# Danya-Is/re2-modification

Measured on AMD Instinct MI355X. Metric: input GB/s (chars matched/sec) on 10-example attack corpus, higher is better.
Workload: dtype u8

## Files before the change

### re2-modification_amd/csrc/walk.h

```cpp
#ifndef MFA_WALK_H
#define MFA_WALK_H

#include <cstddef>
#include <cstdint>

#ifndef WALK_MIN_WAVES
#define WALK_MIN_WAVES 2
#endif

namespace mfa {

constexpr uint32_t WALK_MAX_SEG = 16;
constexpr uint32_t WALK_LDS_BYTES = 160u * 1024u;
constexpr uint32_t CMP_CACHE = 4;
#define MFA_RT_CACHED 2u

constexpr uint32_t walk_W(uint32_t K) { return 2u + 2u * K; }
constexpr uint32_t walk_DW(uint32_t K) { return (1u + 2u * K + 1u) / 2u; }

struct WalkLayout {
    uint32_t K, C, CX;
    bool images_global;
    bool lean;
    uint32_t nm_words;
// ... 19 lines not shown
};
constexpr size_t walk_lds_bytes(uint32_t shared_words, const WalkLayout& l) { return ((size_t)shared_words + 4u * (size_t)l.lds_words()) * sizeof(uint32_t); }

struct WalkArgs {
    const uint8_t*  bytes;
    const uint64_t* offsets;
    uint64_t        n;
    uint8_t*        results;
    const uint64_t* regions;
    const uint32_t* tables;
    uint32_t*       spill;
    unsigned long long* counter;
    uint32_t table_words, shared_words;
    uint32_t n_seg, C, CX, accel, refill;
    uint32_t images_global;
    uint32_t nm_words;
    uint32_t* lean_queue;
    uint32_t* lean_seen;
    uint32_t seg_first[WALK_MAX_SEG + 1];
    uint32_t seg_table[WALK_MAX_SEG];
};

constexpr uint32_t WALK_MAX_K = 9;
enum class WalkKernel { plain, long_k1, stats };

struct WalkLaunch {
    WalkArgs args;
    uint32_t K;
    WalkKernel kernel;
    unsigned grid;
// ... 23 lines not shown
```

### re2-modification_amd/csrc/walk.hip

```cpp
#include <hip/hip_runtime.h>

#include "mfa_internal.h"
#include "walk.h"
#include "walk_core.h"

#ifndef WALK_STATS
#define WALK_STATS 0
#endif
#ifndef WALK_K
#error "compile with -DWALK_K=<cells>"
#endif

namespace mfa {

using namespace mfa_walk;

struct TicketFeeder {
    unsigned long long* counter;
    uint64_t n, first_sid;
    bool first_round = true;
    __device__ __forceinline__ bool take(bool want, uint64_t& sid) {
        const uint32_t lane = threadIdx.x & 63u;
        const unsigned long long wb = __ballot(want);
        unsigned long long first = 0;
// ... 18 lines not shown
    if (!TG) {
        for (uint32_t k = threadIdx.x; k < a.table_words; k += blockDim.x) smem[k] = a.tables[k];
        __syncthreads();
    }
    const WalkLayout lay{(uint32_t)K, a.C, a.CX, a.images_global != 0u, false, WALK_NODE_MAP ? a.nm_words : 0u};
    const uint32_t wave_u = (uint32_t)__builtin_amdgcn_readfirstlane((int)wave);
    WALK_LDS uint32_t* const base = (WALK_LDS uint32_t*)smem + a.shared_words + wave_u * lay.lds_words();
    Store st;
    st.C = a.C; st.CX = a.CX; st.CI = lay.CI();
    st.lv = base + lay.lv(); st.ld = base + lay.ld(); st.sb = base + lay.sb(); st.sa = base + lay.sa();
    WALK_LDS uint64_t* const rtc = (WALK_LDS uint64_t*)(base + lay.rtc());
    st.nm = (WALK_LDS uint8_t*)(base + lay.nm()); st.nm_words = lay.nm_words;
    const uint64_t gwave = (uint64_t)blockIdx.x * 4u + wave_u;
    uint32_t* const g = a.spill + gwave * lay.spill_words();
    st.gv = g + lay.gv(); st.gd = g + lay.gd(); st.gsb = g + lay.gsb(); st.gsa = g + lay.gsa(); st.gq = g + lay.gq();
    Batch b{a.bytes, a.offsets, a.n, a.results, a.regions, a.accel, a.refill, a.n_seg, a.seg_first, a.seg_table, 0u,
            a.lean_queue, reinterpret_cast<uint32_t*>(a.counter + 1)};
    TicketFeeder feed{a.counter, a.n, gwave * 64u};
#if WALK_STATS
    WaveStats ws;
    if (TG) walk_wave<K, REV, TicketFeeder, TablePtrG>(b, a.tables, st, rtc, feed, &ws);
    else walk_wave<K, REV, TicketFeeder, TablePtr>(b, (TablePtr)smem, st, rtc, feed, &ws);
    unsigned long long* out = a.counter + 8;
    const unsigned long long lanev[7] = {ws.dual * 0ull + ws.skipped, ws.probes, ws.hits, ws.steps, ws.spills, ws.strings, 0ull};
    for (int k = 0; k < 6; k++) atomicAdd(&out[k], lanev[k]);
    if ((threadIdx.x & 63u) == 0) {
        const unsigned long long wavev[9] = {ws.iters, ws.dual, ws.t_start, ws.t_byte, ws.t_look, ws.t_plain, ws.t_dual, ws.t_post, ws.t_total};
        for (int k = 0; k < 9; k++) atomicAdd(&out[8 + k], wavev[k]);
        atomicAdd(&out[17], 1ull);
    }
#else
    if (TG) walk_wave<K, REV, TicketFeeder, TablePtrG>(b, a.tables, st, rtc, feed, nullptr);
    else walk_wave<K, REV, TicketFeeder, TablePtr>(b, (TablePtr)smem, st, rtc, feed, nullptr);
#endif
}

struct QueueFeeder {
    const uint32_t* queue;
    uint32_t count;
    unsigned long long* counter;
    __device__ __forceinline__ bool take(bool want, uint64_t& sid) {
        const uint32_t lane = threadIdx.x & 63u;
        const unsigned long long wb = __ballot(want);
        const int leader = __builtin_ctzll(wb);
        unsigned long long first = 0;
        if (lane == (uint32_t)leader) first = atomicAdd(counter, (unsigned long long)__builtin_popcountll(wb));
        const uint32_t at = (uint32_t)__shfl((uint32_t)first, leader) + (uint32_t)__builtin_popcountll(wb & ((1ull << lane) - 1ull));
        const bool got = want && at < count;
// ... 14 lines not shown
        __syncthreads();
    }
    const WalkLayout lay{(uint32_t)K, a.C, a.CX, false, true, WALK_NODE_MAP ? a.nm_words : 0u};
    const uint32_t wave_u = (uint32_t)__builtin_amdgcn_readfirstlane((int)(threadIdx.x >> 6));
    WALK_LDS uint32_t* const base = (WALK_LDS uint32_t*)smem + a.shared_words + wave_u * lay.lds_words();
    Store st;
    st.C = a.C; st.CX = a.CX; st.CI = 0u;
    st.lv = base + lay.lv();
    st.nm = (WALK_LDS uint8_t*)(base + lay.nm()); st.nm_words = lay.nm_words;
    st.ld = nullptr; st.sb = nullptr; st.sa = nullptr;
    const uint64_t gwave = (uint64_t)blockIdx.x * 4u + wave_u;
    uint32_t* const g = a.spill + gwave * lay.spill_words();
    st.gv = g + lay.gv();
    st.gd = nullptr; st.gsb = nullptr; st.gsa = nullptr;
    st.gq = g + lay.gq();
    Batch b{a.bytes, a.offsets, a.n, a.results, nullptr, 0u, a.refill, a.n_seg, a.seg_first, a.seg_table, 0u, nullptr, nullptr};
    QueueFeeder feed{a.lean_queue, count, a.counter + 2};
    if (TG) walk_wave_lean<K, REV, QueueFeeder, TablePtrG>(b, a.tables, st, feed);
    else walk_wave_lean<K, REV, QueueFeeder, TablePtr>(b, (TablePtr)smem, st, feed);
}

#define WALK_CAT2(a, b) a##b
#define WALK_CAT(a, b) WALK_CAT2(a, b)

#if WALK_STATS
int launch_walk_stats(const WalkLaunch& L, void* stream) {
#elif defined(WALK_LONG_LISTS)
int WALK_CAT(launch_walk_long_k, WALK_K)(const WalkLaunch& L, void* stream) {
#else
int WALK_CAT(launch_walk_k, WALK_K)(const WalkLaunch& L, void* stream) {
#endif
// ... 35 lines not shown
```

### re2-modification_amd/csrc/walk_core.h

```cpp
#ifndef MFA_WALK_CORE_H
#define MFA_WALK_CORE_H

#include "../../include/mfa_image_format.h"
#define MFA_SCAN_DEPTH 1
#define MFA_RUN_DEPTH 1
#include "device_common.h"
#include "walk.h"

#ifndef WALK_WV
#define WALK_WV 64u
#endif
#ifndef WALK_DEV
#define WALK_DEV __device__ __forceinline__
#endif
#ifndef WALK_WITH_DUAL
#define WALK_WITH_DUAL 1
#endif
#ifndef WALK_PROBE_PERIODS
#define WALK_PROBE_PERIODS 5u
#endif
#ifndef WALK_NODE_MAP
#define WALK_NODE_MAP 0
#endif
#ifndef WALK_LEAN_MIN_LEN
// ... 10 lines not shown
#define VI_CACC  4u
#define VI_QUAL  8u
#define VI_HASC  (1u << 17)

#define TIE_CARRY 0u
#define TIE_HERE  1u
#define TIE_WAIT  1025u

#ifdef MFA_HOST_EMUL
static unsigned long long g_ev[8];
#define WALK_EV(k) (g_ev[k]++)
WALK_DEV uint32_t wv_lane() { return 0u; }
WALK_DEV uint64_t wv_shfl64(uint64_t v, int) { return v; }
WALK_DEV uint32_t wv_atomic_add(uint32_t* p, uint32_t v) { const uint32_t o = *p; *p = o + v; return o; }
WALK_DEV uint32_t wv_bcast32(uint32_t v, int) { return v; }
template <bool REV>
inline uint32_t coop_run_end_x(const uint8_t* bytes, uint64_t base, uint32_t len, uint32_t i0, uint32_t) {
    if (i0 + 1u >= len) return len;
    auto at = [&](uint32_t j) { return bytes[base + (REV ? (uint64_t)(len - 1u - j) : (uint64_t)j)]; };
    const uint8_t c = at(i0);
    uint32_t j = i0 + 1u;
    while (j < len && at(j) == c) j++;
    return j;
}
inline bool coop_mem_equal_x(const uint8_t* bytes, uint64_t pa, uint64_t pb, uint32_t l, uint32_t) {
    for (uint32_t k = 0; k < l; k++)
        if (bytes[pa + k] != bytes[pb + k]) return false;
    return true;
}
#else
#define WALK_EV(k) ((void)0)
WALK_DEV uint32_t wv_lane() { return threadIdx.x & 63u; }
WALK_DEV uint32_t wv_atomic_add(uint32_t* p, uint32_t v) { return atomicAdd(p, v); }
WALK_DEV uint32_t wv_bcast32(uint32_t v, int L) { return (uint32_t)__shfl((int)v, L); }
WALK_DEV uint64_t wv_shfl64(uint64_t v, int L) { return ((uint64_t)__shfl((uint32_t)(v >> 32), L) << 32) | __shfl((uint32_t)v, L); }
template <bool REV>
__device__ __attribute__((noinline)) uint32_t coop_run_end_x(const uint8_t* bytes, uint64_t base, uint32_t len, uint32_t i0, uint32_t lane) { return coop_run_end<REV>(bytes, base, len, i0, lane); }
__device__ __attribute__((noinline)) bool coop_mem_equal_x(const uint8_t* bytes, uint64_t pa, uint64_t pb, uint32_t l, uint32_t lane) { return coop_mem_equal(bytes, pa, pb, l, lane); }
#endif

#ifdef MFA_HOST_EMUL
#define WALK_LDS
#else
#define WALK_LDS __attribute__((address_space(3)))
#endif
typedef const WALK_LDS uint32_t* TablePtr;
typedef const uint32_t* TablePtrG;

struct WIn {
    const uint8_t*  bytes;
    uint64_t        total16;
    const uint64_t* regions;
    WALK_LDS uint64_t* rtc;
    uint64_t base;
    uint32_t len, sid;
    uint64_t blk;
    uint32_t w0, w1, w2, w3;
    uint32_t run_lo, run_hi, run_ch;
    uint32_t per_lo, per_hi, per_q;
    uint32_t prev_lo, prev_hi, prev_q;
    uint32_t dual_p;
    uint32_t rt_cnt;
    uint32_t rq;
    uint32_t rq_a, rq_b, rq_l;
    uint32_t cq_n;
};

WALK_DEV void w_drop_window(WIn& in) { in.blk = MFA_NO_WINDOW; }
WALK_DEV void w_reset(WIn& in, uint64_t base, uint32_t len, uint32_t sid) {
    in.base = base; in.len = len; in.sid = sid;
    w_drop_window(in);
    in.run_lo = in.run_hi = 0; in.run_ch = 0x100u;
    in.per_lo = in.per_hi = 0; in.per_q = 0; in.dual_p = 0;
    in.prev_lo = in.prev_hi = 0; in.prev_q = 0;
    in.rt_cnt = 0; in.rq = 0; in.rq_a = in.rq_b = in.rq_l = 0; in.cq_n = 0;
}

WALK_DEV void w_rt_attach(WIn& in, uint32_t& warm, const uint4 a, const uint4 b) {
    if (in.regions == nullptr) return;
    const uint32_t lane = wv_lane();
// ... 539 lines not shown
        }
}
#endif

template <int K, class TP>
WALK_DEV void ee_decode(TP T, uint32_t at, bool p, uint32_t& e0, uint32_t& actions, uint32_t& cm, uint32_t& com, uint32_t& rdm) {
    e0 = p ? T[at] : 0u;
    const uint32_t e1 = p ? T[at + 1] : 0u;
    if (Lay<K>::EEW == 2) {
        actions = e1 & 0xfffu; cm = (e1 >> 12) & 0x3fu; com = (e1 >> 18) & 0x3fu; rdm = (e1 >> 24) & 0x3fu;
    } else {
        const uint32_t e2 = p ? T[at + 2] : 0u;
        actions = e1 & 0x3ffffu; cm = (e1 >> 18) & 0x1ffu; com = e2 & 0x1ffu; rdm = (e2 >> 9) & 0x1ffu;
    }
}

template <class U, int K>
WALK_DEV void frame_state(const Ent<U, K>& E, U pos, uint32_t cm, uint32_t com, uint32_t rdm, Ent<U, K>& s) {
#pragma unroll
    for (int c = 0; c < K; c++) {
        const bool created = (cm >> c) & 1u;
        s.S[c] = sel(created, pos, E.S[c]);
        s.L[c] = sel(created, konst<U>(0u), E.L[c]);
        s.F[c] = created ? (F_PRESENT | F_UNI | (((com >> c) & 1u) ? F_OPEN : 0u)) : E.F[c];
        if ((rdm >> c) & 1u) s.F[c] |= F_READ;
    }
}

#ifndef WALK_STEP_ATTR
#define WALK_STEP_ATTR WALK_DEV
#endif
template <class U, int K, bool REV, class TP>
WALK_STEP_ATTR void walk_step(const Store& st, TP T, const Aut& au, WIn& in, uint32_t cur, uint32_t n_cur, uint32_t& n_next,
                        const U i, const U len, const uint32_t ch, const bool final_pass, const bool active, const bool dual_lane,
                        bool& accept, bool& fits, tb_t& TB, uint32_t& shape) {
    StepCtx<U, K> cx{st, cur ^ 1u, 0u, dual_lane, fits, TB, {}};
    cx.keys.seen = 0ull;
    uint32_t sh = 0u;
#pragma unroll
    for (uint32_t k = 0; k < KeyCache<U>::N; k++) cx.keys.id[k] = 0xffffffffu;
    const uint32_t cls = (active && !final_pass) ? (T[au.cmap() + ((ch & 0xffu) >> 2)] >> (8u * (ch & 3u))) & 0xffu : 0u;
    for (uint32_t e = 0; __any(active && e < n_cur); e++) {
        const bool have = active && e < n_cur;
        if (have) WALK_EV(0);
        Ent<U, K> E;
        load_entry<U, K>(st, cur, have ? e : 0u, dual_lane && have, E);
        const U pos = have ? posof(E.P, cx.TB) : konst<U>(0u);
        bool live = have && ge(pos, i, cx.TB);
        if (REV) {
            if (live) {
                U need = konst<U>(0u);
#pragma unroll
                for (int c = 0; c < K; c++)
                    if ((E.F[c] & F_PRESENT) && ((E.F[c] & F_OPEN) || !(E.F[c] & F_READ))) need = add(need, E.L[c]);
                live = le(need, sub(len, i), cx.TB);
            }
        }
        const bool here = live && !final_pass && eq(pos, i, cx.TB);
        const bool wait = live && !final_pass && !here;
        const uint32_t vi = have ? T[au.vinfo() + E.vid] : 0u;
        const uint32_t node = E.vid >> au.vbits();
#if WALK_NODE_MAP
        if (have) {
            WALK_LDS uint8_t* const mp = st.nm + nm_at(node);
            if (*mp == (uint8_t)((cur << 7) | e)) *mp = 0xffu;
        }
#endif
        if (have) {
            const uint32_t ahead = val(pos) - val(i);
            sh = ((sh << 7) | (sh >> 25)) ^ (E.vid * 4u + (ahead < 3u ? ahead : 3u) + 0x9e37u);
        }
        if ((vi & VI_EPS) && live && !accept && eq(pos, len, cx.TB)) accept = true;
        {
            const bool carry = wait && (vi & VI_QUAL) != 0u;
            if (__any(carry)) { Ent<U, K> t = E; insert<U, K>(cx, carry, E.vid, au.vbits(), E.P, TIE_CARRY, t); }
        }
        if (__any(here)) {
            const uint32_t bl = here ? T[au.vb() + E.vid * au.nc() + cls] : 0u;
            const uint32_t bbeg = bl >> 12, bcnt = bl & 0xfffu;
            for (uint32_t j = 0; __any(j < bcnt); j++) {
                const bool p = here && j < bcnt;
                if (p) WALK_EV(1);
                uint32_t e0, actions, cm, com, rdm;
                ee_decode<K, TP>(T, au.ee() + (bbeg + j) * Lay<K>::EEW, p, e0, actions, cm, com, rdm);
                const uint32_t tvid = e0 >> 9, tfn = (e0 >> 5) & 15u, cell = (e0 >> 1) & 15u;
                Ent<U, K> t = E;
                if (__any(p && (cm | rdm) != 0u)) frame_state<U, K>(E, pos, cm, com, rdm, t);
                const bool lit = p && (e0 & 1u) == 0u, rd = p && (e0 & 1u) != 0u;
                if (__any(lit)) {
                    apply_actions<U, K>(t, actions, lit, i, konst<U>(1u), true, ch, cx.TB);
                    insert<U, K>(cx, lit, tvid, au.vbits(), mkp(add(i, konst<U>(1u)), tfn), TIE_HERE + node, t);
                }
                if (__any(rd)) {
                    U vs = konst<U>(0u), vl = konst<U>(0u);
                    uint32_t vf = 0u;
#pragma unroll
                    for (int c = 0; c < K; c++)
                        if ((uint32_t)c == cell) { vs = t.S[c]; vl = t.L[c]; vf = t.F[c]; }
                    const bool ok = cell_read<REV, U>(st, in, rd, i, ch, vs, vl, vf, cx.TB);
                    if (__any(ok)) {
                        apply_actions<U, K>(t, actions, ok, i, vl, (vf & F_UNI) != 0u, (vf >> 8) & 0xffu, cx.TB);
                        insert<U, K>(cx, ok, tvid, au.vbits(), mkp(add(i, vl), tfn), TIE_HERE + node, t);
                    }
                }
            }
        }
        const bool late = live && !here;
        if ((vi & VI_CACC) && late && !accept && eq(pos, len, cx.TB)) accept = true;
        if (__any(wait && (vi & VI_HASC) != 0u)) {
            const uint32_t cl = (wait && (vi & VI_HASC) != 0u) ? T[au.vc() + E.vid] : 0u;
            const uint32_t cbeg = cl >> 12, ccnt = cl & 0xfffu;
            for (uint32_t j = 0; __any(j < ccnt); j++) {
                const bool p = wait && j < ccnt;
                if (p) WALK_EV(6);
                uint32_t e0, actions, cm, com, rdm;
                ee_decode<K, TP>(T, au.ee() + (cbeg + j) * Lay<K>::EEW, p, e0, actions, cm, com, rdm);
                Ent<U, K> t;
                frame_state<U, K>(E, pos, cm, com, 0u, t);
                insert<U, K>(cx, p, e0 >> 9, au.vbits(), mkp(pos, (e0 >> 5) & 15u), TIE_WAIT + node, t);
            }
        }
    }
    n_next = cx.n_next; fits = cx.fits; TB = cx.TB; shape = sh;
}

template <int K> WALK_DEV void sb_rd_words(const Store& st, uint32_t e, uint32_t (&w)[Lay<K>::W]) {
    if (e < st.CI) {
        const WALK_LDS uint32_t* p = st.sb + (e * Lay<K>::W) * WALK_WV + wv_lane();
#pragma unroll
        for (uint32_t k = 0; k < Lay<K>::W; k++) w[k] = p[k * WALK_WV];
    } else {
        const uint32_t* p = st.gsb + (size_t)((e - st.CI) * Lay<K>::W) * WALK_WV + wv_lane();
#pragma unroll
        for (uint32_t k = 0; k < Lay<K>::W; k++) w[k] = p[k * WALK_WV];
    }
}
template <int K> WALK_DEV void sb_wr_words(const Store& st, uint32_t e, const uint32_t (&w)[Lay<K>::W]) {
    if (e < st.CI) {
// ... 133 lines not shown
    const uint64_t* regions;
    uint32_t accel;
    uint32_t refill;
    uint32_t n_seg;
    const uint32_t* seg_first;
    const uint32_t* seg_table;
    uint32_t reserved;
    uint32_t* lean_queue;
    uint32_t* lean_count;
};

struct WaveStats {
    unsigned long long iters = 0, dual = 0, skipped = 0, probes = 0, hits = 0, steps = 0, spills = 0;
    unsigned long long t_start = 0, t_byte = 0, t_look = 0, t_plain = 0, t_dual = 0, t_post = 0, t_total = 0;
    unsigned long long strings = 0;
#ifdef MFA_HOST_EMUL
    unsigned long long hist[80] = {0};
#endif
};
#ifdef MFA_HOST_EMUL
WALK_DEV unsigned long long wv_clock() { return 0ull; }
#else
WALK_DEV unsigned long long wv_clock() { return __builtin_readcyclecounter(); }
#endif

struct ProbeCtl {
    uint32_t w;
    WALK_DEV uint32_t get(uint32_t sh, uint32_t bits) const { return (w >> sh) & ((1u << bits) - 1u); }
    WALK_DEV void put(uint32_t sh, uint32_t bits, uint32_t v) { w = (w & ~(((1u << bits) - 1u) << sh)) | ((v & ((1u << bits) - 1u)) << sh); }
    WALK_DEV void reset() { w = 0u; set_pp(1u); backoff_reset(); }
// ... 32 lines not shown
    }
    WALK_DEV uint32_t period(uint32_t q, uint32_t pmin) const {
        const uint32_t c = (uint32_t)(h >> 60);
        uint32_t m = 0u;
#pragma unroll
        for (uint32_t p = 1; p <= HIST_MAX_P; p++)
            if (((h ^ (h >> (5u * p))) & 1023ull) == 0ull) m |= 1u << p;
        const uint64_t lo = 0xffffull | (0x5555ull << 16) | (0x9249ull << 32) | (0x1111ull << 48), hi = 0x8421ull | (0x1041ull << 16) | (0x4081ull << 32) | (0x0101ull << 48);
        m &= (uint32_t)((q <= 4u ? lo : hi) >> (((q - 1u) & 3u) << 4)) & 0xffffu;
        m &= c >= 3u ? (1u << (c - 1u)) - 2u : 0u;
        m &= ~((1u << (pmin < 16u ? pmin : 16u)) - 1u);
        return m ? (uint32_t)__builtin_ctz(m) : 0u;
    }
};

template <int K, bool REV, class Feeder, class TP>
WALK_DEV void walk_wave(const Batch& b, TP T, const Store& st, WALK_LDS uint64_t* rt_cache, Feeder& feed, WaveStats* stats) {
    WIn in;
    in.bytes = b.bytes; in.total16 = (b.offsets[b.n] + 15u) & ~(uint64_t)15; in.regions = b.regions; in.rtc = rt_cache;
    w_reset(in, 0, 0, 0);
    in.w0 = in.w1 = in.w2 = in.w3 = 0;
    bool active = false, exhausted = false, accept = false;
    uint32_t i = 0, len = 0;
    uint32_t probe_at = 0;
    ProbeCtl P;
    P.reset();
    ShapeHist hist;
    hist.reset();
    tb_t TBacc = tb_init();
    bool fits = true, stable = false, patient = false;
    uint32_t cur = 0, n_cur = 0, sb_n = 0, warm = 0;
    Aut au;
    aut_load(au, T, 0u);
    const unsigned long long tm_begin = stats ? wv_clock() : 0ull;
    for (;;) {
        unsigned long long tm = stats ? wv_clock() : 0ull;
// ... 99 lines not shown
        }
        WALK_LAP(t_look);
        uint32_t n_next = 0, shape = 0;
        tb_t TB = tb_init();
        const bool p2 = P.phase() == 2u;
        const bool accept_before = accept, fits_before = fits;
        in.cq_n = 0u;
        for (;;) {
            n_next = 0; TB = tb_init(); accept = accept_before; fits = fits_before;
            if (WALK_WITH_DUAL && __any(p2)) {
                if (stats) stats->dual++;
                const Dual di{i, (int32_t)P.pp()}, dlen{len, 0};
                in.dual_p = p2 ? P.pp() : 0u;
                (void)lt(di, Dual{p2 ? in.per_hi : i + 1u, 0}, TB);
                (void)eq(di, dlen, TB);
                walk_step<Dual, K, REV, TP>(st, T, au, in, cur, n_cur, n_next, di, dlen, ch, final_pass, active, p2, accept, fits, TB, shape);
                in.dual_p = 0u;
                WALK_LAP(t_dual);
            } else {
                bool f2 = true;
                walk_step<uint32_t, K, REV, TP>(st, T, au, in, cur, n_cur, n_next, i, len, ch, final_pass, active, false, accept, f2, TB, shape);
                WALK_LAP(t_plain);
            }
            if (!__any(active && in.rq != 0u)) break;
            answer_requests<REV>(st, in, active);
#if WALK_NODE_MAP
            map_forget<K>(st, au.vbits(), cur ^ 1u, active, n_next);
#endif
        }
        cur ^= 1u;
        if (active) { n_cur = n_next; hist.push(shape); }
        const bool any_next = n_next != 0u;
        if (stats && active && n_cur > st.C) stats->spills++;
#ifdef MFA_HOST_EMUL
        if (stats && active) stats->hist[n_cur < 79u ? n_cur : 79u]++;
#endif
// ... 70 lines not shown
            }
        }
        if (active) {
            const bool done = accept || final_pass || !any_next;
            i++;
            if (stats) stats->steps++;
            if (done) {
                b.results[in.sid] = (warm == 0x9e3779b9u && len == 0xffffffffu) ? 3 : (accept ? 1 : 0);
                active = false; P.set_phase(0u); P.set_chain(0u); n_cur = 0u;
                if (stats) stats->strings++;
            }
        }
        WALK_LAP(t_post);
    }
#undef WALK_LAP
    if (stats) stats->t_total += wv_clock() - tm_begin;
}

template <int K, bool REV, class Feeder, class TP>
WALK_DEV void walk_wave_lean(const Batch& b, TP T, const Store& st, Feeder& feed) {
    WIn in;
    in.bytes = b.bytes; in.total16 = (b.offsets[b.n] + 15u) & ~(uint64_t)15; in.regions = nullptr; in.rtc = nullptr;
    w_reset(in, 0, 0, 0);
    in.w0 = in.w1 = in.w2 = in.w3 = 0;
    bool active = false, exhausted = false, accept = false;
    uint32_t i = 0, len = 0, cur = 0, n_cur = 0;
    Aut au;
    aut_load(au, T, 0u);
    for (;;) {
        {
            const bool want = !active && !exhausted;
            const unsigned long long wantb = __ballot(want);
            if (wantb && ((uint32_t)__builtin_popcountll(wantb) >= b.refill || !__any(active))) {
                uint64_t s = 0;
                const bool got = feed.take(want, s);
                if (want) {
                    if (!got) exhausted = true;
                    else {
                        const uint64_t o0 = b.offsets[s], o1 = b.offsets[s + 1];
                        len = (uint32_t)(o1 - o0);
                        w_reset(in, o0, len, (uint32_t)s);
                        uint32_t seg = 0;
                        for (uint32_t k = 1; k < b.n_seg; k++)
                            if (s >= b.seg_first[k]) seg = k;
                        aut_load(au, T, b.n_seg ? b.seg_table[seg] : 0u);
                        i = 0; accept = false; active = true;
#if WALK_NODE_MAP
                        for (uint32_t k = 0; k < st.nm_words; k++) reinterpret_cast<WALK_LDS uint32_t*>(st.nm)[k * WALK_WV + wv_lane()] = 0xffffffffu;
#endif
                        n_cur = 1;
                        Ent<uint32_t, K> e0;
                        e0.P = 0u; e0.vid = aut_start(T, au);
#pragma unroll
                        for (int c = 0; c < K; c++) { e0.S[c] = 0u; e0.L[c] = 0u; e0.F[c] = 0u; }
                        bool f2 = true;
                        store_entry<uint32_t, K>(st, cur, 0u, e0, 0u, f2);
                    }
                }
            }
        }
        if (!__any(active)) break;
        const bool final_pass = (i == len);
        uint32_t ch = 0x100u;
        if (active && !final_pass) ch = w_stream_byte<REV>(in, i);
        uint32_t n_next = 0, shape = 0;
        const bool accept_before = accept;
        in.cq_n = 0u;
        for (;;) {
            n_next = 0; accept = accept_before;
            tb_t TB = tb_init();
            bool f2 = true;
            walk_step<uint32_t, K, REV, TP>(st, T, au, in, cur, n_cur, n_next, i, len, ch, final_pass, active, false, accept, f2, TB, shape);
            if (!__any(active && in.rq != 0u)) break;
            answer_requests<REV>(st, in, active);
#if WALK_NODE_MAP
            map_forget<K>(st, au.vbits(), cur ^ 1u, active, n_next);
#endif
        }
        cur ^= 1u;
        if (active) {
            n_cur = n_next;
            const bool done = accept || final_pass || n_next == 0u;
            i++;
            if (done) { b.results[in.sid] = accept ? 1 : 0; active = false; n_cur = 0u; }
        }
    }
}
// ... 5 lines not shown
```

### re2-modification_amd/csrc/walk_launch.hip

```cpp
#include <hip/hip_runtime.h>

#include <algorithm>
#include <cstdio>
#include <cstdlib>
#include <cstring>
#include <map>
#include <new>
#include <string>
#include <vector>

#include "dfa_mixed.h"
#include "mfa_internal.h"
#include "walk.h"

namespace mfa {

int launch_walk(const WalkPlanInput& p, const uint32_t* d_tables, int n_cus, const uint8_t* d_bytes, const uint64_t* d_offsets, uint64_t n,
                uint8_t* d_results, const uint64_t* d_regions, uint32_t n_seg, const uint32_t* seg_first, const uint32_t* seg_table,
                uint32_t** d_spill, size_t* spill_bytes, unsigned long long* d_counter, void* stream, LeanHint* lean, void* wait_event) {
    if (n == 0) { if (wait_event) HIP_TRY(hipStreamWaitEvent((hipStream_t)stream, (hipEvent_t)wait_event, 0)); return MFA_OK; }
    const WalkKnobs kn = walk_knobs();
    Lean decision = d_regions != nullptr && kn.accel && kn.lean != 0 ? Lean::on : Lean::off;
    LeanHint next;
    const bool hinted = decision == Lean::on && lean != nullptr;
// ... 32 lines not shown

void lean_hint_free(LeanHint& h) {
    if (h.h_seen) (void)hipHostFree(h.h_seen);
    h.h_seen = nullptr;
}

void walk_print_stats(unsigned long long* d_counter, const char* tag) {
    unsigned long long h[32] = {0};
    if (hipMemcpy(h, d_counter, sizeof h, hipMemcpyDeviceToHost) != hipSuccess) return;
    const unsigned long long* o = h + 8;
    const double tot = (double)o[16] > 0 ? (double)o[16] : 1.0;
    fprintf(stderr, "%s stats: %llu waves, %llu strings, wave-iterations %llu (dual %llu), lane steps %llu, skipped %llu, probes %llu (hits %llu), spill steps %llu\n", tag,
            o[17], o[5], o[8], o[9], o[3], o[0], o[1], o[2], o[4]);
    fprintf(stderr, "%s stats: cycles per wave-iteration %.0f; share: string start %.1f%%, byte %.1f%%, region look-up %.1f%%, plain step %.1f%%, dual step %.1f%%, book-keeping %.1f%%\n", tag,
            tot / (double)(o[8] ? o[8] : 1), 100.0 * o[10] / tot, 100.0 * o[11] / tot, 100.0 * o[12] / tot, 100.0 * o[13] / tot, 100.0 * o[14] / tot, 100.0 * o[15] / tot);
}

}

using namespace mfa;

constexpr uint32_t MIX_TIMINGS = 32;

struct mfa_mixed {
    std::vector<mfa_image*> images;
    std::vector<uint32_t>   words;
    std::vector<uint32_t>   block_at;
    uint32_t K = 1, max_live = 1;
    bool reversed = false, table_ok = true;
    std::vector<uint8_t>    is_dfa, dfa_eligible, dfa_tables;
// ... 374 lines not shown
```

### re2-modification_amd/csrc/walk_plan.h

```cpp
#ifndef MFA_WALK_PLAN_H
#define MFA_WALK_PLAN_H

#include <algorithm>
#include <cmath>
#include <cstdint>
#include <cstdlib>
#include <string>
#include <vector>

#include "../../include/mfa_hip.h"
#include "walk.h"

namespace mfa {

inline int env_int(const char* name, int dflt) {
    const char* e = getenv(name);
    return e && *e ? atoi(e) : dflt;
}
inline bool env_is_off(const char* name) { const char* e = getenv(name); return e && e[0] == '0'; }
inline bool regions_enabled() { return !env_is_off("MFA_REGIONS") && !env_is_off("MFA_ACCEL"); }

inline int walk_mode() {
    const char* e = getenv("MFA_WALK");
    return !e ? 0 : e[0] == 't' ? 1 : e[0] == 'j' ? 2 : 0;
}

struct WalkPlanInput { uint32_t K, max_live; bool reversed; uint32_t table_words; };

struct LeanHint {
    uint32_t* h_seen = nullptr;
    uint32_t quiet = 0, launches = 0;
};
enum class Lean { off, on, probe };

struct WalkKnobs {
    bool tables_global, images_global, accel, long_lists, stats;
    int refill, want_c, wgs, waves_per_cu, grid_pct, spill_mb, lean;
};
inline WalkKnobs walk_knobs() {
    WalkKnobs k;
    k.tables_global = getenv("MFA_WALK_TABLES_GLOBAL") != nullptr;
    k.images_global = env_int("MFA_WALK_IMAGES_GLOBAL", 0) != 0;
    k.accel = !env_is_off("MFA_ACCEL");
    k.long_lists = env_int("MFA_WALK_LONG", 1) != 0;
    k.stats = getenv("MFA_WALK_STATS") != nullptr;
    k.refill = std::max(1, std::min(64, env_int("MFA_WALK_REFILL", 1)));
    k.want_c = env_int("MFA_WALK_C", 0);
    k.wgs = env_int("MFA_WALK_WGS", 0);
    k.waves_per_cu = env_int("MFA_WALK_WAVES_PER_CU", 0);
    k.grid_pct = env_int("MFA_WALK_GRID_PCT", 100);
    k.spill_mb = std::max(1, env_int("MFA_WALK_SPILL_MB", 2048));
    k.lean = env_int("MFA_WALK_LEAN", 1);
    return k;
}

inline Lean lean_decide(uint32_t seen, LeanHint& h, const WalkKnobs& kn) {
    h.quiet = seen == 1u ? h.quiet + 1u : 0u;
    Lean d = Lean::on;
    if (h.quiet >= 1u && kn.lean != 2) d = (h.launches & 31u) != 0u ? Lean::off : Lean::probe;
    h.launches++;
    return d;
}

inline int plan_walk(const WalkPlanInput& p, const WalkKnobs& kn, uint64_t n, int n_cus, uint32_t n_seg, Lean lean, WalkLaunch& L) {
    if (n_seg == 0 || n_seg > WALK_MAX_SEG || n > 0xffffffffull) return MFA_ERR_INVALID_ARG;
    L = WalkLaunch{};
    WalkArgs& a = L.args;
    a.n = n; a.n_seg = n_seg;
    a.table_words = p.table_words;
    a.shared_words = (p.table_words + 63u) & ~63u;
    const size_t lds_max = WALK_LDS_BYTES / 4u;
    L.tables_global = a.shared_words > lds_max / 3u || kn.tables_global;
    if (L.tables_global) a.shared_words = 0;
    a.accel = kn.accel ? 1u : 0u;
    a.refill = (uint32_t)kn.refill;
    a.images_global = kn.images_global ? 1u : 0u;
    L.K = p.K; L.reversed = p.reversed;
    const bool long_lists = p.K == 1 && p.max_live > 16u && p.max_live < 128u && kn.long_lists && !kn.stats;
    L.kernel = kn.stats && p.K == 1 ? WalkKernel::stats : long_lists ? WalkKernel::long_k1 : WalkKernel::plain;
    a.nm_words = long_lists ? (p.max_live + 1u + 3u) / 4u : 0u;
    const auto layout = [&](uint32_t C, bool lean_walk) { return WalkLayout{p.K, C, p.max_live > C ? p.max_live - C : 1u, kn.images_global, lean_walk, a.nm_words}; };
    const auto lds_words = [&](uint32_t C) { return (size_t)a.shared_words + 4u * (size_t)layout(C, false).lds_words(); };
    const uint64_t cus = (uint64_t)(n_cus > 0 ? n_cus : 256), want = (n + 255) / 256;
    const uint32_t wgs_goal = kn.wgs != 0 ? (uint32_t)kn.wgs : want <= cus ? 1u : 2u;
    uint32_t C = std::max(1u, std::min(p.max_live, kn.want_c > 0 ? (uint32_t)kn.want_c : 8u));
    while (C > 1 && kn.want_c <= 0 && lds_words(C) > lds_max / wgs_goal) C--;
    while (C > 1 && lds_words(C) > lds_max) C--;
    if (lds_words(C) > lds_max) return MFA_ERR_UNSUPPORTED;
    const WalkLayout full = layout(C, false), lean_lay = layout(C, true);
// ... 164 lines not shown
```

Baseline: 5270.

## Add wave-uniform scalar step path when all lanes share state and class

Before each step, the code checks with ballots whether every active lane has the same automaton, the same byte class and the same list of vertex ids. If they do, it runs a specialised path that broadcasts the ids and reads table entries with readfirstlane, so the loads become scalar and the loop bounds are uniform. The goal is to cut divergent vector table lookups and per-lane loop control. The main kernel keeps the general path unless WALK_UNIFORM_MAIN is set, so only the lean kernel takes the new path by default, and it pays for the uniformity check on every step even when lanes differ.

Result: no change. 5265 (-0.1%).

```diff
diff --git a/re2-modification_amd/csrc/walk.h b/re2-modification_amd/csrc/walk.h
--- a/re2-modification_amd/csrc/walk.h
+++ b/re2-modification_amd/csrc/walk.h
@@ -57,6 +57,7 @@
     uint32_t table_words, shared_words;
     uint32_t n_seg, C, CX, accel, refill;
     uint32_t images_global;
+    uint32_t flags;
     uint32_t nm_words;
     uint32_t* lean_queue;
     uint32_t* lean_seen;
diff --git a/re2-modification_amd/csrc/walk.hip b/re2-modification_amd/csrc/walk.hip
--- a/re2-modification_amd/csrc/walk.hip
+++ b/re2-modification_amd/csrc/walk.hip
@@ -6,6 +6,9 @@
 
 #ifndef WALK_STATS
 #define WALK_STATS 0
+#endif
+#ifndef WALK_UNIFORM_MAIN
+#define WALK_UNIFORM_MAIN WALK_STATS
 #endif
 #ifndef WALK_K
 #error "compile with -DWALK_K=<cells>"
@@ -56,13 +59,13 @@
     const uint64_t gwave = (uint64_t)blockIdx.x * 4u + wave_u;
     uint32_t* const g = a.spill + gwave * lay.spill_words();
     st.gv = g + lay.gv(); st.gd = g + lay.gd(); st.gsb = g + lay.gsb(); st.gsa = g + lay.gsa(); st.gq = g + lay.gq();
-    Batch b{a.bytes, a.offsets, a.n, a.results, a.regions, a.accel, a.refill, a.n_seg, a.seg_first, a.seg_table, 0u,
+    Batch b{a.bytes, a.offsets, a.n, a.results, a.regions, a.accel, a.refill, a.n_seg, a.seg_first, a.seg_table, a.flags & 1u,
             a.lean_queue, reinterpret_cast<uint32_t*>(a.counter + 1)};
     TicketFeeder feed{a.counter, a.n, gwave * 64u};
 #if WALK_STATS
     WaveStats ws;
-    if (TG) walk_wave<K, REV, TicketFeeder, TablePtrG>(b, a.tables, st, rtc, feed, &ws);
-    else walk_wave<K, REV, TicketFeeder, TablePtr>(b, (TablePtr)smem, st, rtc, feed, &ws);
+    if (TG) walk_wave<K, REV, TicketFeeder, TablePtrG, WALK_UNIFORM_MAIN != 0>(b, a.tables, st, rtc, feed, &ws);
+    else walk_wave<K, REV, TicketFeeder, TablePtr, WALK_UNIFORM_MAIN != 0>(b, (TablePtr)smem, st, rtc, feed, &ws);
     unsigned long long* out = a.counter + 8;
     const unsigned long long lanev[7] = {ws.dual * 0ull + ws.skipped, ws.probes, ws.hits, ws.steps, ws.spills, ws.strings, 0ull};
     for (int k = 0; k < 6; k++) atomicAdd(&out[k], lanev[k]);
@@ -70,10 +73,12 @@
         const unsigned long long wavev[9] = {ws.iters, ws.dual, ws.t_start, ws.t_byte, ws.t_look, ws.t_plain, ws.t_dual, ws.t_post, ws.t_total};
         for (int k = 0; k < 9; k++) atomicAdd(&out[8 + k], wavev[k]);
         atomicAdd(&out[17], 1ull);
+        atomicAdd(&out[18], ws.ent_uni);
+        atomicAdd(&out[19], ws.ent_gen);
     }
 #else
-    if (TG) walk_wave<K, REV, TicketFeeder, TablePtrG>(b, a.tables, st, rtc, feed, nullptr);
-    else walk_wave<K, REV, TicketFeeder, TablePtr>(b, (TablePtr)smem, st, rtc, feed, nullptr);
+    if (TG) walk_wave<K, REV, TicketFeeder, TablePtrG, WALK_UNIFORM_MAIN != 0>(b, a.tables, st, rtc, feed, nullptr);
+    else walk_wave<K, REV, TicketFeeder, TablePtr, WALK_UNIFORM_MAIN != 0>(b, (TablePtr)smem, st, rtc, feed, nullptr);
 #endif
 }
 
@@ -118,7 +123,7 @@
     st.gv = g + lay.gv();
     st.gd = nullptr; st.gsb = nullptr; st.gsa = nullptr;
     st.gq = g + lay.gq();
-    Batch b{a.bytes, a.offsets, a.n, a.results, nullptr, 0u, a.refill, a.n_seg, a.seg_first, a.seg_table, 0u, nullptr, nullptr};
+    Batch b{a.bytes, a.offsets, a.n, a.results, nullptr, 0u, a.refill, a.n_seg, a.seg_first, a.seg_table, a.flags & 1u, nullptr, nullptr};
     QueueFeeder feed{a.lean_queue, count, a.counter + 2};
     if (TG) walk_wave_lean<K, REV, QueueFeeder, TablePtrG>(b, a.tables, st, feed);
     else walk_wave_lean<K, REV, QueueFeeder, TablePtr>(b, (TablePtr)smem, st, feed);
diff --git a/re2-modification_amd/csrc/walk_core.h b/re2-modification_amd/csrc/walk_core.h
--- a/re2-modification_amd/csrc/walk_core.h
+++ b/re2-modification_amd/csrc/walk_core.h
@@ -48,6 +48,8 @@
 WALK_DEV uint64_t wv_shfl64(uint64_t v, int) { return v; }
 WALK_DEV uint32_t wv_atomic_add(uint32_t* p, uint32_t v) { const uint32_t o = *p; *p = o + v; return o; }
 WALK_DEV uint32_t wv_bcast32(uint32_t v, int) { return v; }
+WALK_DEV uint32_t wv_read_lane(uint32_t v, int) { return v; }
+template <bool UNI> WALK_DEV uint32_t wv_uni(uint32_t v) { return v; }
 template <bool REV>
 inline uint32_t coop_run_end_x(const uint8_t* bytes, uint64_t base, uint32_t len, uint32_t i0, uint32_t) {
     if (i0 + 1u >= len) return len;
@@ -68,10 +70,14 @@
 WALK_DEV uint32_t wv_atomic_add(uint32_t* p, uint32_t v) { return atomicAdd(p, v); }
 WALK_DEV uint32_t wv_bcast32(uint32_t v, int L) { return (uint32_t)__shfl((int)v, L); }
 WALK_DEV uint64_t wv_shfl64(uint64_t v, int L) { return ((uint64_t)__shfl((uint32_t)(v >> 32), L) << 32) | __shfl((uint32_t)v, L); }
+WALK_DEV uint32_t wv_read_lane(uint32_t v, int L) { return (uint32_t)__builtin_amdgcn_readlane((int)v, L); }
+template <bool UNI> WALK_DEV uint32_t wv_uni(uint32_t v) { return UNI ? (uint32_t)__builtin_amdgcn_readfirstlane((int)v) : v; }
 template <bool REV>
 __device__ __attribute__((noinline)) uint32_t coop_run_end_x(const uint8_t* bytes, uint64_t base, uint32_t len, uint32_t i0, uint32_t lane) { return coop_run_end<REV>(bytes, base, len, i0, lane); }
 __device__ __attribute__((noinline)) bool coop_mem_equal_x(const uint8_t* bytes, uint64_t pa, uint64_t pb, uint32_t l, uint32_t lane) { return coop_mem_equal(bytes, pa, pb, l, lane); }
 #endif
+
+template <bool UNI> WALK_DEV bool wv_any(bool c) { return UNI ? c : __any(c) != 0; }
 
 #ifdef MFA_HOST_EMUL
 #define WALK_LDS
@@ -98,6 +104,7 @@
     uint32_t rq;
     uint32_t rq_a, rq_b, rq_l;
     uint32_t cq_n;
+    uint32_t ev_uni, ev_gen;
 };
 
 WALK_DEV void w_drop_window(WIn& in) { in.blk = MFA_NO_WINDOW; }
@@ -667,6 +674,17 @@
         actions = e1 & 0x3ffffu; cm = (e1 >> 18) & 0x1ffu; com = e2 & 0x1ffu; rdm = (e2 >> 9) & 0x1ffu;
     }
 }
+template <int K, class TP>
+WALK_DEV void ee_decode_uni(TP T, uint32_t at, uint32_t& e0, uint32_t& actions, uint32_t& cm, uint32_t& com, uint32_t& rdm) {
+    e0 = wv_uni<true>(T[at]);
+    const uint32_t e1 = wv_uni<true>(T[at + 1]);
+    if (Lay<K>::EEW == 2) {
+        actions = e1 & 0xfffu; cm = (e1 >> 12) & 0x3fu; com = (e1 >> 18) & 0x3fu; rdm = (e1 >> 24) & 0x3fu;
+    } else {
+        const uint32_t e2 = wv_uni<true>(T[at + 2]);
+        actions = e1 & 0x3ffffu; cm = (e1 >> 18) & 0x1ffu; com = e2 & 0x1ffu; rdm = (e2 >> 9) & 0x1ffu;
+    }
+}
 
 template <class U, int K>
 WALK_DEV void frame_state(const Ent<U, K>& E, U pos, uint32_t cm, uint32_t com, uint32_t rdm, Ent<U, K>& s) {
@@ -680,19 +698,93 @@
     }
 }
 
-#ifndef WALK_STEP_ATTR
-#define WALK_STEP_ATTR WALK_DEV
-#endif
-template <class U, int K, bool REV, class TP>
-WALK_STEP_ATTR void walk_step(const Store& st, TP T, const Aut& au, WIn& in, uint32_t cur, uint32_t n_cur, uint32_t& n_next,
-                        const U i, const U len, const uint32_t ch, const bool final_pass, const bool active, const bool dual_lane,
-                        bool& accept, bool& fits, tb_t& TB, uint32_t& shape) {
-    StepCtx<U, K> cx{st, cur ^ 1u, 0u, dual_lane, fits, TB, {}};
-    cx.keys.seen = 0ull;
+#ifdef WALK_NO_UNIFORM
+#define WALK_UNIFORM 0
+#else
+#define WALK_UNIFORM 1
+#endif
+#ifndef WALK_UNIFORM_DUAL
+#define WALK_UNIFORM_DUAL 1
+#endif
+template <class U> struct UniStep { static constexpr bool on = WALK_UNIFORM != 0; };
+template <> struct UniStep<Dual> { static constexpr bool on = WALK_UNIFORM != 0 && WALK_UNIFORM_DUAL != 0; };
+
+template <bool UNI, class U, int K, bool REV, class TP>
+WALK_DEV void step_entry(StepCtx<U, K>& cx, TP T, const Aut& au, WIn& in, const Ent<U, K>& E, const uint32_t vid, const uint32_t cls,
+                         const uint32_t cur, const uint32_t e, const U pos, const U i, const U len, const uint32_t ch,
+                         const bool have, const bool live, const bool final_pass, bool& accept) {
+    const Store& st = cx.st;
+    const bool here = live && !final_pass && eq(pos, i, cx.TB);
+    const bool wait = live && !final_pass && !here;
+    const uint32_t vi = (UNI || have) ? wv_uni<UNI>(T[au.vinfo() + vid]) : 0u;
+    const uint32_t node = vid >> au.vbits();
+#if WALK_NODE_MAP
+    if (have) {
+        WALK_LDS uint8_t* const mp = st.nm + nm_at(node);
+        if (*mp == (uint8_t)((cur << 7) | e)) *mp = 0xffu;
+    }
+#endif
+    if ((vi & VI_EPS) && live && !accept && eq(pos, len, cx.TB)) accept = true;
+    {
+        const bool carry = wait && (vi & VI_QUAL) != 0u;
+        if (__any(carry)) { Ent<U, K> t = E; insert<U, K>(cx, carry, vid, au.vbits(), E.P, TIE_CARRY, t); }
+    }
+    if (__any(here)) {
+        const uint32_t bl = (UNI || here) ? wv_uni<UNI>(T[au.vb() + vid * au.nc() + cls]) : 0u;
+        const uint32_t bbeg = bl >> 12, bcnt = bl & 0xfffu;
+        for (uint32_t j = 0; wv_any<UNI>(j < bcnt); j++) {
+            const bool p = here && j < bcnt;
+            if (p) WALK_EV(1);
+            uint32_t e0, actions, cm, com, rdm;
+            if (UNI) ee_decode_uni<K, TP>(T, au.ee() + (bbeg + j) * Lay<K>::EEW, e0, actions, cm, com, rdm);
+            else ee_decode<K, TP>(T, au.ee() + (bbeg + j) * Lay<K>::EEW, p, e0, actions, cm, com, rdm);
+            const uint32_t tvid = e0 >> 9, tfn = (e0 >> 5) & 15u, cell = (e0 >> 1) & 15u;
+            Ent<U, K> t = E;
+            if (wv_any<UNI>(p && (cm | rdm) != 0u)) frame_state<U, K>(E, pos, cm, com, rdm, t);
+            const bool lit = p && (e0 & 1u) == 0u, rd = p && (e0 & 1u) != 0u;
+            if (__any(lit)) {
+                apply_actions<U, K>(t, actions, lit, i, konst<U>(1u), true, ch, cx.TB);
+                insert<U, K>(cx, lit, tvid, au.vbits(), mkp(add(i, konst<U>(1u)), tfn), TIE_HERE + node, t);
+            }
+            if (__any(rd)) {
+                U vs = konst<U>(0u), vl = konst<U>(0u);
+                uint32_t vf = 0u;
+#pragma unroll
+                for (int c = 0; c < K; c++)
+                    if ((uint32_t)c == cell) { vs = t.S[c]; vl = t.L[c]; vf = t.F[c]; }
+                const bool ok = cell_read<REV, U>(st, in, rd, i, ch, vs, vl, vf, cx.TB);
+                if (__any(ok)) {
+                    apply_actions<U, K>(t, actions, ok, i, vl, (vf & F_UNI) != 0u, (vf >> 8) & 0xffu, cx.TB);
+                    insert<U, K>(cx, ok, tvid, au.vbits(), mkp(add(i, vl), tfn), TIE_HERE + node, t);
+                }
+            }
+        }
+    }
+    const bool late = live && !here;
+    if ((vi & VI_CACC) && late && !accept && eq(pos, len, cx.TB)) accept = true;
+    const bool wc = wait && (vi & VI_HASC) != 0u;
+    if (__any(wc)) {
+        const uint32_t cl = (UNI || wc) ? wv_uni<UNI>(T[au.vc() + vid]) : 0u;
+        const uint32_t cbeg = cl >> 12, ccnt = cl & 0xfffu;
+        for (uint32_t j = 0; wv_any<UNI>(j < ccnt); j++) {
+            const bool p = wc && j < ccnt;
+            if (p) WALK_EV(6);
+            uint32_t e0, actions, cm, com, rdm;
+            if (UNI) ee_decode_uni<K, TP>(T, au.ee() + (cbeg + j) * Lay<K>::EEW, e0, actions, cm, com, rdm);
+            else ee_decode<K, TP>(T, au.ee() + (cbeg + j) * Lay<K>::EEW, p, e0, actions, cm, com, rdm);
+            Ent<U, K> t;
+            frame_state<U, K>(E, pos, cm, com, 0u, t);
+            insert<U, K>(cx, p, e0 >> 9, au.vbits(), mkp(pos, (e0 >> 5) & 15u), TIE_WAIT + node, t);
+        }
+    }
+}
+
+template <bool UNI, class U, int K, bool REV, class TP>
+WALK_DEV void step_entries(StepCtx<U, K>& cx, TP T, const Aut& au, WIn& in, const uint32_t cls, const uint32_t cur, const uint32_t n_cur,
+                           const U i, const U len, const uint32_t ch, const bool final_pass, const bool active, const bool dual_lane,
+                           bool& accept, uint32_t& shape) {
+    const Store& st = cx.st;
     uint32_t sh = 0u;
-#pragma unroll
-    for (uint32_t k = 0; k < KeyCache<U>::N; k++) cx.keys.id[k] = 0xffffffffu;
-    const uint32_t cls = (active && !final_pass) ? (T[au.cmap() + ((ch & 0xffu) >> 2)] >> (8u * (ch & 3u))) & 0xffu : 0u;
     for (uint32_t e = 0; __any(active && e < n_cur); e++) {
         const bool have = active && e < n_cur;
         if (have) WALK_EV(0);
@@ -709,72 +801,57 @@
                 live = le(need, sub(len, i), cx.TB);
             }
         }
-        const bool here = live && !final_pass && eq(pos, i, cx.TB);
-        const bool wait = live && !final_pass && !here;
-        const uint32_t vi = have ? T[au.vinfo() + E.vid] : 0u;
-        const uint32_t node = E.vid >> au.vbits();
-#if WALK_NODE_MAP
-        if (have) {
-            WALK_LDS uint8_t* const mp = st.nm + nm_at(node);
-            if (*mp == (uint8_t)((cur << 7) | e)) *mp = 0xffu;
-        }
-#endif
         if (have) {
             const uint32_t ahead = val(pos) - val(i);
             sh = ((sh << 7) | (sh >> 25)) ^ (E.vid * 4u + (ahead < 3u ? ahead : 3u) + 0x9e37u);
         }
-        if ((vi & VI_EPS) && live && !accept && eq(pos, len, cx.TB)) accept = true;
-        {
-            const bool carry = wait && (vi & VI_QUAL) != 0u;
-            if (__any(carry)) { Ent<U, K> t = E; insert<U, K>(cx, carry, E.vid, au.vbits(), E.P, TIE_CARRY, t); }
-        }
-        if (__any(here)) {
-            const uint32_t bl = here ? T[au.vb() + E.vid * au.nc() + cls] : 0u;
-            const uint32_t bbeg = bl >> 12, bcnt = bl & 0xfffu;
-            for (uint32_t j = 0; __any(j < bcnt); j++) {
-                const bool p = here && j < bcnt;
-                if (p) WALK_EV(1);
-                uint32_t e0, actions, cm, com, rdm;
-                ee_decode<K, TP>(T, au.ee() + (bbeg + j) * Lay<K>::EEW, p, e0, actions, cm, com, rdm);
-                const uint32_t tvid = e0 >> 9, tfn = (e0 >> 5) & 15u, cell = (e0 >> 1) & 15u;
-                Ent<U, K> t = E;
-                if (__any(p && (cm | rdm) != 0u)) frame_state<U, K>(E, pos, cm, com, rdm, t);
-                const bool lit = p && (e0 & 1u) == 0u, rd = p && (e0 & 1u) != 0u;
-                if (__any(lit)) {
-                    apply_actions<U, K>(t, actions, lit, i, konst<U>(1u), true, ch, cx.TB);
-                    insert<U, K>(cx, lit, tvid, au.vbits(), mkp(add(i, konst<U>(1u)), tfn), TIE_HERE + node, t);
-                }
-                if (__any(rd)) {
-                    U vs = konst<U>(0u), vl = konst<U>(0u);
-                    uint32_t vf = 0u;
-#pragma unroll
-                    for (int c = 0; c < K; c++)
-                        if ((uint32_t)c == cell) { vs = t.S[c]; vl = t.L[c]; vf = t.F[c]; }
-                    const bool ok = cell_read<REV, U>(st, in, rd, i, ch, vs, vl, vf, cx.TB);
-                    if (__any(ok)) {
-                        apply_actions<U, K>(t, actions, ok, i, vl, (vf & F_UNI) != 0u, (vf >> 8) & 0xffu, cx.TB);
-                        insert<U, K>(cx, ok, tvid, au.vbits(), mkp(add(i, vl), tfn), TIE_HERE + node, t);
-                    }
-                }
-            }
-        }
-        const bool late = live && !here;
-        if ((vi & VI_CACC) && late && !accept && eq(pos, len, cx.TB)) accept = true;
-        if (__any(wait && (vi & VI_HASC) != 0u)) {
-            const uint32_t cl = (wait && (vi & VI_HASC) != 0u) ? T[au.vc() + E.vid] : 0u;
-            const uint32_t cbeg = cl >> 12, ccnt = cl & 0xfffu;
-            for (uint32_t j = 0; __any(j < ccnt); j++) {
-                const bool p = wait && j < ccnt;
-                if (p) WALK_EV(6);
-                uint32_t e0, actions, cm, com, rdm;
-                ee_decode<K, TP>(T, au.ee() + (cbeg + j) * Lay<K>::EEW, p, e0, actions, cm, com, rdm);
-                Ent<U, K> t;
-                frame_state<U, K>(E, pos, cm, com, 0u, t);
-                insert<U, K>(cx, p, e0 >> 9, au.vbits(), mkp(pos, (e0 >> 5) & 15u), TIE_WAIT + node, t);
-            }
-        }
-    }
-    n_next = cx.n_next; fits = cx.fits; TB = cx.TB; shape = sh;
+        const uint32_t vid = UNI ? wv_read_lane(E.vid, __builtin_ctzll(__ballot(have))) : E.vid;
+        if (UNI) in.ev_uni++; else in.ev_gen++;
+        step_entry<UNI, U, K, REV, TP>(cx, T, au, in, E, vid, cls, cur, e, pos, i, len, ch, have, live, final_pass, accept);
+    }
+    shape = sh;
+}
+
+#ifndef WALK_STEP_ATTR
+#define WALK_STEP_ATTR WALK_DEV
+#endif
+template <class U, int K, bool REV, class TP, bool UNIW>
+WALK_STEP_ATTR void walk_step(const Store& st, TP T, const Aut& au, WIn& in, uint32_t cur, uint32_t n_cur, uint32_t& n_next,
+                        const U i, const U len, const uint32_t ch, const bool final_pass, const bool active, const bool dual_lane,
+                        bool& accept, bool& fits, tb_t& TB, uint32_t& shape, const bool uni_on) {
+    StepCtx<U, K> cx{st, cur ^ 1u, 0u, dual_lane, fits, TB, {}};
+    cx.keys.seen = 0ull;
+#pragma unroll
+    for (uint32_t k = 0; k < KeyCache<U>::N; k++) cx.keys.id[k] = 0xffffffffu;
+    const uint32_t cls = (active && !final_pass) ? (T[au.cmap() + ((ch & 0xffu) >> 2)] >> (8u * (ch & 3u))) & 0xffu : 0u;
+    bool step_uni = false;
+    Aut au_u{0u, 0u};
+    uint32_t cls_u = 0u;
+    if (UNIW && UniStep<U>::on && uni_on) {
+        const unsigned long long ab = __ballot(active);
+        if (ab) {
+            const int la = __builtin_ctzll(ab);
+            au_u.at = wv_read_lane(au.at, la); au_u.dims = wv_read_lane(au.dims, la);
+            const unsigned long long cb = __ballot(active && !final_pass);
+            cls_u = wv_read_lane(cls, cb ? __builtin_ctzll(cb) : la);
+            bool differ = active && (au.at != au_u.at || (!final_pass && cls != cls_u));
+            for (uint32_t e = 0; __any(active && e < n_cur); e++) {
+                const bool have = active && e < n_cur;
+                const uint32_t v = rd_v<K>(st, cur, have ? e : 0u, 1) & 0xffffu;
+                if (have && v != wv_read_lane(v, __builtin_ctzll(__ballot(have)))) differ = true;
+            }
+            step_uni = !__any(differ);
+        }
+    }
+    if (UNIW && UniStep<U>::on && step_uni)
+        step_entries<true, U, K, REV, TP>(cx, T, au_u, in, cls_u, cur, n_cur, i, len, ch, final_pass, active, dual_lane, accept, shape);
+    else {
+#if defined(MFA_HOST_EMUL) && defined(WALK_TRAP_GENERAL)
+        if (uni_on && active) { fprintf(stderr, "walk_step: the general path was taken by a wave of one lane\n"); abort(); }
+#endif
+        step_entries<false, U, K, REV, TP>(cx, T, au, in, cls, cur, n_cur, i, len, ch, final_pass, active, dual_lane, accept, shape);
+    }
+    n_next = cx.n_next; fits = cx.fits; TB = cx.TB;
 }
 
 template <int K> WALK_DEV void sb_rd_words(const Store& st, uint32_t e, uint32_t (&w)[Lay<K>::W]) {
@@ -938,6 +1015,7 @@
     unsigned long long iters = 0, dual = 0, skipped = 0, probes = 0, hits = 0, steps = 0, spills = 0;
     unsigned long long t_start = 0, t_byte = 0, t_look = 0, t_plain = 0, t_dual = 0, t_post = 0, t_total = 0;
     unsigned long long strings = 0;
+    unsigned long long ent_uni = 0, ent_gen = 0;
 #ifdef MFA_HOST_EMUL
     unsigned long long hist[80] = {0};
 #endif
@@ -1000,12 +1078,14 @@
     }
 };
 
-template <int K, bool REV, class Feeder, class TP>
+template <int K, bool REV, class Feeder, class TP, bool UNIW = true>
 WALK_DEV void walk_wave(const Batch& b, TP T, const Store& st, WALK_LDS uint64_t* rt_cache, Feeder& feed, WaveStats* stats) {
     WIn in;
     in.bytes = b.bytes; in.total16 = (b.offsets[b.n] + 15u) & ~(uint64_t)15; in.regions = b.regions; in.rtc = rt_cache;
     w_reset(in, 0, 0, 0);
     in.w0 = in.w1 = in.w2 = in.w3 = 0;
+    in.ev_uni = in.ev_gen = 0u;
+    const bool uni_on = (b.reserved & 1u) == 0u;
     bool active = false, exhausted = false, accept = false;
     uint32_t i = 0, len = 0;
     uint32_t probe_at = 0;
@@ -1135,12 +1215,12 @@
                 in.dual_p = p2 ? P.pp() : 0u;
                 (void)lt(di, Dual{p2 ? in.per_hi : i + 1u, 0}, TB);
                 (void)eq(di, dlen, TB);
-                walk_step<Dual, K, REV, TP>(st, T, au, in, cur, n_cur, n_next, di, dlen, ch, final_pass, active, p2, accept, fits, TB, shape);
+                walk_step<Dual, K, REV, TP, UNIW>(st, T, au, in, cur, n_cur, n_next, di, dlen, ch, final_pass, active, p2, accept, fits, TB, shape, uni_on);
                 in.dual_p = 0u;
                 WALK_LAP(t_dual);
             } else {
                 bool f2 = true;
-                walk_step<uint32_t, K, REV, TP>(st, T, au, in, cur, n_cur, n_next, i, len, ch, final_pass, active, false, accept, f2, TB, shape);
+                walk_step<uint32_t, K, REV, TP, UNIW>(st, T, au, in, cur, n_cur, n_next, i, len, ch, final_pass, active, false, accept, f2, TB, shape, uni_on);
                 WALK_LAP(t_plain);
             }
             if (!__any(active && in.rq != 0u)) break;
@@ -1241,7 +1321,7 @@
         WALK_LAP(t_post);
     }
 #undef WALK_LAP
-    if (stats) stats->t_total += wv_clock() - tm_begin;
+    if (stats) { stats->t_total += wv_clock() - tm_begin; stats->ent_uni += in.ev_uni; stats->ent_gen += in.ev_gen; }
 }
 
 template <int K, bool REV, class Feeder, class TP>
@@ -1250,6 +1330,8 @@
     in.bytes = b.bytes; in.total16 = (b.offsets[b.n] + 15u) & ~(uint64_t)15; in.regions = nullptr; in.rtc = nullptr;
     w_reset(in, 0, 0, 0);
     in.w0 = in.w1 = in.w2 = in.w3 = 0;
+    in.ev_uni = in.ev_gen = 0u;
+    const bool uni_on = (b.reserved & 1u) == 0u;
     bool active = false, exhausted = false, accept = false;
     uint32_t i = 0, len = 0, cur = 0, n_cur = 0;
     Aut au;
@@ -1267,10 +1349,10 @@
                         const uint64_t o0 = b.offsets[s], o1 = b.offsets[s + 1];
                         len = (uint32_t)(o1 - o0);
                         w_reset(in, o0, len, (uint32_t)s);
-                        uint32_t seg = 0;
+                        uint32_t at = b.n_seg ? b.seg_table[0] : 0u;
                         for (uint32_t k = 1; k < b.n_seg; k++)
-                            if (s >= b.seg_first[k]) seg = k;
-                        aut_load(au, T, b.n_seg ? b.seg_table[seg] : 0u);
+                            if (s >= b.seg_first[k]) at = b.seg_table[k];
+                        aut_load(au, T, at);
                         i = 0; accept = false; active = true;
 #if WALK_NODE_MAP
                         for (uint32_t k = 0; k < st.nm_words; k++) reinterpret_cast<WALK_LDS uint32_t*>(st.nm)[k * WALK_WV + wv_lane()] = 0xffffffffu;
@@ -1297,7 +1379,7 @@
             n_next = 0; accept = accept_before;
             tb_t TB = tb_init();
             bool f2 = true;
-            walk_step<uint32_t, K, REV, TP>(st, T, au, in, cur, n_cur, n_next, i, len, ch, final_pass, active, false, accept, f2, TB, shape);
+            walk_step<uint32_t, K, REV, TP, true>(st, T, au, in, cur, n_cur, n_next, i, len, ch, final_pass, active, false, accept, f2, TB, shape, uni_on);
             if (!__any(active && in.rq != 0u)) break;
             answer_requests<REV>(st, in, active);
 #if WALK_NODE_MAP
diff --git a/re2-modification_amd/csrc/walk_launch.hip b/re2-modification_amd/csrc/walk_launch.hip
--- a/re2-modification_amd/csrc/walk_launch.hip
+++ b/re2-modification_amd/csrc/walk_launch.hip
@@ -70,6 +70,7 @@
             o[17], o[5], o[8], o[9], o[3], o[0], o[1], o[2], o[4]);
     fprintf(stderr, "%s stats: cycles per wave-iteration %.0f; share: string start %.1f%%, byte %.1f%%, region look-up %.1f%%, plain step %.1f%%, dual step %.1f%%, book-keeping %.1f%%\n", tag,
             tot / (double)(o[8] ? o[8] : 1), 100.0 * o[10] / tot, 100.0 * o[11] / tot, 100.0 * o[12] / tot, 100.0 * o[13] / tot, 100.0 * o[14] / tot, 100.0 * o[15] / tot);
+    fprintf(stderr, "%s stats: list entries %llu uniform, %llu general, uniform share %.3f\n", tag, o[18], o[19], (double)o[18] / (double)(o[18] + o[19] ? o[18] + o[19] : 1));
 }
 
 }
diff --git a/re2-modification_amd/csrc/walk_plan.h b/re2-modification_amd/csrc/walk_plan.h
--- a/re2-modification_amd/csrc/walk_plan.h
+++ b/re2-modification_amd/csrc/walk_plan.h
@@ -34,7 +34,7 @@
 enum class Lean { off, on, probe };
 
 struct WalkKnobs {
-    bool tables_global, images_global, accel, long_lists, stats;
+    bool tables_global, images_global, accel, long_lists, stats, uniform;
     int refill, want_c, wgs, waves_per_cu, grid_pct, spill_mb, lean;
 };
 inline WalkKnobs walk_knobs() {
@@ -51,6 +51,7 @@
     k.grid_pct = env_int("MFA_WALK_GRID_PCT", 100);
     k.spill_mb = std::max(1, env_int("MFA_WALK_SPILL_MB", 2048));
     k.lean = env_int("MFA_WALK_LEAN", 1);
+    k.uniform = !env_is_off("MFA_WALK_UNIFORM");
     return k;
 }
 
@@ -73,6 +74,7 @@
     L.tables_global = a.shared_words > lds_max / 3u || kn.tables_global;
     if (L.tables_global) a.shared_words = 0;
     a.accel = kn.accel ? 1u : 0u;
+    a.flags = kn.uniform ? 0u : 1u;
     a.refill = (uint32_t)kn.refill;
     a.images_global = kn.images_global ? 1u : 0u;
     L.K = p.K; L.reversed = p.reversed;
```
